# chanchanchan97/ICAFusion

Measured on AMD Instinct MI355X. Metric: RGB/IR image-pairs/sec (two-stream forward + NMS), higher is better.
Workload: dtype bf16

## Files before the change

### icafusion_amd/csrc/detect.hip

```cpp
#pragma clang fp contract(off)
#include "icaf_common.h"
#include "stream_core.h"
#include <cstdlib>

namespace icaf {

struct Anchors { float v[16]; };
int conv_prepare(const icaf_conv_args* a, ConvP& p);

struct DetectDiv { FastDiv no, nx, ny, na; };

template <bool I32>
__global__ __launch_bounds__(256) void detect_decode_kernel(const float* __restrict__ p, int ldp, float* __restrict__ z,
                                                            float* __restrict__ logits, float* __restrict__ raw, int B, int ny, int nx,
                                                            int na, int no, long long rows_total, long long row_offset, float stride,
                                                            Anchors anc, DetectDiv dv) {
    const long long total = (long long)B * na * ny * nx * no;
    for (long long e = (long long)blockIdx.x * blockDim.x + threadIdx.x; e < total; e += (long long)gridDim.x * blockDim.x) {
        int o, x, y, a, b;
        if constexpr (I32) {
            unsigned int q, r;
            fd_divmod((unsigned int)e, dv.no, q, r);
            o = (int)r;
            fd_divmod(q, dv.nx, q, r);
            x = (int)r;
            fd_divmod(q, dv.ny, q, r);
            y = (int)r;
            fd_divmod(q, dv.na, q, r);
            a = (int)r;
            b = (int)q;
        } else {
            o = (int)(e % no);
            const long long idx = e / no;
            x = (int)(idx % nx);
            long long t = idx / nx;
            y = (int)(t % ny);
            t /= ny;
            a = (int)(t % na);
            b = (int)(t / na);
        }
        const float v = p[(((long long)b * ny + y) * nx + x) * ldp + a * no + o];
        const long long row = (long long)b * rows_total + row_offset + ((long long)a * ny + y) * nx + x;
        if (raw) raw[e] = v;
        if (logits && o >= 5) logits[row * (no - 5) + (o - 5)] = v;
        const float sg = 1.0f / (1.0f + expf(-v));
        float out = sg;
        if (o == 0) out = ((sg * 2.0f - 0.5f) + (float)x) * stride;
        else if (o == 1) out = ((sg * 2.0f - 0.5f) + (float)y) * stride;
        else if (o == 2 || o == 3) {
            float an = anc.v[o - 2];
#pragma unroll
            for (int i = 1; i < 8; ++i) an = (a == i) ? (o == 2 ? anc.v[2 * i] : anc.v[2 * i + 1]) : an;
            const float d = sg * 2.0f;
            out = (d * d) * an;
        }
        z[row * no + o] = out;
    }
}

template <int NA, int NO>
__global__ __launch_bounds__(256) void detect_pixel_kernel(const float* __restrict__ p, int ldp, float* __restrict__ z,
                                                           float* __restrict__ logits, float* __restrict__ raw, int B, int ny, int nx,
                                                           long long rows_total, long long row_offset, float stride, Anchors anc,
                                                           FastDiv dnx, FastDiv dny) {
    constexpr int NV = NA * NO;
    const unsigned int total = (unsigned int)B * ny * nx;
    for (unsigned int pix = blockIdx.x * blockDim.x + threadIdx.x; pix < total; pix += gridDim.x * blockDim.x) {
        unsigned int t, x, b, y;
        fd_divmod(pix, dnx, t, x);
        fd_divmod(t, dny, b, y);
        const float* src = p + (long long)pix * ldp;
        float v[NV];
#pragma unroll
        for (int i = 0; i < NV; i += 2) {
            const float2 q = *(const float2*)(src + i);
            v[i] = q.x; v[i + 1] = q.y;
        }
#pragma unroll
        for (int a = 0; a < NA; ++a) {
            const long long cell = ((long long)a * ny + y) * nx + x;
            const long long row = (long long)b * rows_total + row_offset + cell;
            float o[NO];
#pragma unroll
            for (int k = 0; k < NO; ++k) {
                const float sg = 1.0f / (1.0f + expf(-v[a * NO + k]));
                float out = sg;
                if (k == 0) out = ((sg * 2.0f - 0.5f) + (float)x) * stride;
                else if (k == 1) out = ((sg * 2.0f - 0.5f) + (float)y) * stride;
                else if (k == 2 || k == 3) {
                    const float d = sg * 2.0f;
                    out = (d * d) * anc.v[2 * a + (k - 2)];
                }
                o[k] = out;
            }
            float* zr = z + row * NO;
#pragma unroll
            for (int k = 0; k < NO; k += 2) *(float2*)(zr + k) = float2{o[k], o[k + 1]};
            if (raw) {
                float* rr = raw + (((long long)b * NA) * ny * nx + cell) * NO;
#pragma unroll
                for (int k = 0; k < NO; k += 2) *(float2*)(rr + k) = float2{v[a * NO + k], v[a * NO + k + 1]};
            }
            if (logits) {
#pragma unroll
                for (int k = 5; k < NO; ++k) logits[row * (NO - 5) + (k - 5)] = v[a * NO + k];
            }
        }
    }
}

template <int NA, int NO>
static int launch_detect_pixel(const float* p, int ldp, float* z, float* logits, float* raw, int B, int ny, int nx, long long rows_total,
                               long long row_offset, float stride, const Anchors& anc, hipStream_t s) {
    const long long pixels = (long long)B * ny * nx;
    long long blocks = (pixels + 255) / 256;
    if (blocks > 256 * 32) blocks = 256 * 32;
    hipLaunchKernelGGL((detect_pixel_kernel<NA, NO>), dim3((unsigned)blocks), dim3(256), 0, s, p, ldp, z, logits, raw, B, ny, nx, rows_total,
                       row_offset, stride, anc, make_fastdiv((unsigned)nx), make_fastdiv((unsigned)ny));
    ICAF_LAUNCH_CHECK();
    return ICAF_OK;
}

template <int NA, int NO>
struct DetectEpi {
    static constexpr int SO = 64 * 4 + 16;
    float* z; float* logits; float* raw;
    int M, ny, nx; long long rows_total, row_offset; float stride; Anchors anc; FastDiv dnx, dny;
    template <int TM>
    __device__ __forceinline__ void stage(const f32x16 (&acc)[TM], const f32x4 (&bq)[4], unsigned char* stg, int row0, int col0, int l31, int hi, int, int) const {
#pragma unroll
        for (int qd = 0; qd < 4; ++qd) {
            const int nl = col0 + 8 * qd + 4 * hi;
#pragma unroll
            for (int b = 0; b < TM; ++b) {
                const int ml = row0 + b * 32 + l31;
                f32x4 v;
#pragma unroll
                for (int j = 0; j < 4; ++j) v[j] = acc[b][4 * qd + j] + bq[qd][j];
                *(f32x4*)(stg + ml * SO + nl * 4) = v;
            }
        }
    }
    __device__ __forceinline__ void flush(const unsigned char* stg, int m0, int n0, int tid) const {
        if (tid >= 128 * NA) return;
        const int row = tid / NA, a = tid - row * NA;
        const unsigned int pix = (unsigned int)(m0 + row);
        if ((int)pix >= M) return;
        unsigned int t, x, b, y;
        fd_divmod(pix, dnx, t, x);
        fd_divmod(t, dny, b, y);
        const float* src = (const float*)(stg + row * SO) + a * NO;
        float v[NO];
#pragma unroll
        for (int k = 0; k < NO; k += 2) { const float2 q2 = *(const float2*)(src + k); v[k] = q2.x; v[k + 1] = q2.y; }
        const long long cell = ((long long)a * ny + y) * nx + x;
        const long long zrow = (long long)b * rows_total + row_offset + cell;
        float o[NO];
#pragma unroll
        for (int k = 0; k < NO; ++k) {
            const float sg = 1.0f / (1.0f + expf(-v[k]));
            float out = sg;
            if (k == 0) out = ((sg * 2.0f - 0.5f) + (float)x) * stride;
            else if (k == 1) out = ((sg * 2.0f - 0.5f) + (float)y) * stride;
            else if (k == 2 || k == 3) {
                const float d = sg * 2.0f;
                out = (d * d) * anc.v[2 * a + (k - 2)];
            }
            o[k] = out;
        }
        float* zr = z + zrow * NO;
#pragma unroll
        for (int k = 0; k < NO; k += 2) *(float2*)(zr + k) = float2{o[k], o[k + 1]};
        if (raw) {
            float* rr = raw + (((long long)b * NA) * ny * nx + cell) * NO;
#pragma unroll
            for (int k = 0; k < NO; k += 2) *(float2*)(rr + k) = float2{v[k], v[k + 1]};
        }
        if (logits) {
#pragma unroll
            for (int k = 5; k < NO; ++k) logits[zrow * (NO - 5) + (k - 5)] = v[k];
        }
    }
};

template <int DT, int NA, int NO>
__global__ __launch_bounds__(512) void detect_conv_kernel(const ConvP p, const DetectEpi<NA, NO> epi) {
    stream_gemm<DT, 64, 1>(p, epi);
}

template <int DT, int NA, int NO>
static int launch_detect_conv(const ConvP& p, const DetectEpi<NA, NO>& epi, hipStream_t s) {
    constexpr int LDS = 3 * (128 + 64) * 128 + 128 * DetectEpi<NA, NO>::SO;
    ConvP q = p;
    q.mtiles = (p.M + 127) / 128;
    q.ntiles = 1;
    q.nchunks = p.K / 64;
    int dev = 0, cus = 256;
    ICAF_HIP(hipGetDevice(&dev));
    ICAF_HIP(hipDeviceGetAttribute(&cus, hipDeviceAttributeMultiprocessorCount, dev));
    const int grid = cus & ~7;
    ICAF_LDS_OPTIN((detect_conv_kernel<DT, NA, NO>), LDS);
    detect_conv_kernel<DT, NA, NO><<<dim3((unsigned)grid, 1, 1), dim3(512), LDS, s>>>(q, epi);
    ICAF_LAUNCH_CHECK();
    return ICAF_OK;
}

}

using namespace icaf;

enum { DETECT_PIXEL = 0, DETECT_ELEMENT = 1 };

static int detect_select(const float* p, int ldp, const float* z, const float* raw, int B, int ny, int nx, int na, int no) {
    const bool aligned = ldp % 2 == 0 && ((uintptr_t)p & 7) == 0 && ((uintptr_t)z & 7) == 0 && (!raw || ((uintptr_t)raw & 7) == 0);
    const bool pixel = na == 3 && (no == 6 || no == 8 || no == 14) && aligned && (long long)B * ny * nx < (1ll << 31) && !g_opt.detect_elementwise;
    return pixel ? DETECT_PIXEL : DETECT_ELEMENT;
}

extern "C" int icaf_detect_decode_kernel(const float* p, int ldp, const float* z, const float* raw, int B, int ny, int nx, int na, int no,
                                         int* kernel) {
    if (!p || !z || !kernel) return fail(ICAF_ERR_ARG, "icaf_detect_decode_kernel: null pointer");
    if (na < 1 || na > 8 || no < 6 || ldp < na * no) return fail(ICAF_ERR_ARG, "icaf_detect_decode_kernel: bad na/no/ldp");
    if (B < 1 || ny < 1 || nx < 1) return fail(ICAF_ERR_ARG, "icaf_detect_decode_kernel: empty level");
    *kernel = detect_select(p, ldp, z, raw, B, ny, nx, na, no);
    return ICAF_OK;
}

extern "C" int icaf_detect_decode(const float* p, int ldp, float* z, float* logits, float* raw, int B, int ny, int nx, int na, int no,
                                  long long rows_total, long long row_offset, float stride, const float* anchors_px, icaf_stream_t s) {
    if (!p || !z || !anchors_px) return fail(ICAF_ERR_ARG, "icaf_detect_decode: null pointer");
    if (na < 1 || na > 8 || no < 6 || ldp < na * no) return fail(ICAF_ERR_ARG, "icaf_detect_decode: bad na/no/ldp");
    if (row_offset + (long long)na * ny * nx > rows_total) return fail(ICAF_ERR_ARG, "icaf_detect_decode: level does not fit in z");
    Anchors anc;
    for (int i = 0; i < 16; ++i) anc.v[i] = i < 2 * na ? anchors_px[i] : 0.0f;
    const long long cells = (long long)B * na * ny * nx * no;
    long long blocks = (cells + 255) / 256;
    if (blocks > 256 * 32) blocks = 256 * 32;
    if (B < 1 || ny < 1 || nx < 1) return fail(ICAF_ERR_ARG, "icaf_detect_decode: empty level");
    if (detect_select(p, ldp, z, raw, B, ny, nx, na, no) == DETECT_PIXEL) {
        if (no == 6) return launch_detect_pixel<3, 6>(p, ldp, z, logits, raw, B, ny, nx, rows_total, row_offset, stride, anc, S(s));
        if (no == 8) return launch_detect_pixel<3, 8>(p, ldp, z, logits, raw, B, ny, nx, rows_total, row_offset, stride, anc, S(s));
        if (no == 14) return launch_detect_pixel<3, 14>(p, ldp, z, logits, raw, B, ny, nx, rows_total, row_offset, stride, anc, S(s));
    }
    const DetectDiv dv{make_fastdiv((unsigned)no), make_fastdiv((unsigned)nx), make_fastdiv((unsigned)ny), make_fastdiv((unsigned)na)};
    if (cells < (1ll << 31))
        hipLaunchKernelGGL(detect_decode_kernel<true>, dim3((unsigned)blocks), dim3(256), 0, S(s), p, ldp, z, logits, raw, B, ny, nx, na,
                           no, rows_total, row_offset, stride, anc, dv);
    else
        hipLaunchKernelGGL(detect_decode_kernel<false>, dim3((unsigned)blocks), dim3(256), 0, S(s), p, ldp, z, logits, raw, B, ny, nx, na,
                           no, rows_total, row_offset, stride, anc, dv);
    ICAF_LAUNCH_CHECK();
    return ICAF_OK;
}

extern "C" int icaf_detect_conv(const icaf_conv_args* a, float* z, float* logits, float* raw, int na, int no, long long rows_total,
                                long long row_offset, float stride, const float* anchors_px, icaf_stream_t s) {
    if (!a || !z || !anchors_px) return fail(ICAF_ERR_ARG, "icaf_detect_conv: null pointer");
    ConvP p;
    int st = conv_prepare(a, p);
    if (st) return st;
    if (a->dtype == ICAF_F32) return fail(ICAF_ERR_UNSUPPORTED, "icaf_detect_conv: 16-bit feature maps (the fp32 build runs icaf_conv2d + icaf_detect_decode)");
    if (a->kh != 1 || a->kw != 1 || a->sh != 1 || a->sw != 1 || a->ph || a->pw || a->groups != 1 || a->res || a->pre || a->w2 || a->act != ICAF_ACT_NONE)
        return fail(ICAF_ERR_ARG, "icaf_detect_conv: a plain 1x1 convolution without activation is expected");
    if ((a->Cin * 2) % 128 || p.x_bytes == 0) return fail(ICAF_ERR_UNSUPPORTED, "icaf_detect_conv: Cin * 2 bytes must be a multiple of 128 (Cin = %d)", a->Cin);
    if (na != 3 || (no != 6 && no != 8 && no != 14) || a->Cout != na * no) return fail(ICAF_ERR_UNSUPPORTED, "icaf_detect_conv: built for 3 anchors, no in {6, 8, 14} (na = %d, no = %d, Cout = %d)", na, no, a->Cout);
    if (row_offset + (long long)na * a->Ho * a->Wo > rows_total) return fail(ICAF_ERR_ARG, "icaf_detect_conv: level does not fit in z");
    if (((uintptr_t)z & 7) || (raw && ((uintptr_t)raw & 7))) return fail(ICAF_ERR_ARG, "icaf_detect_conv: z / raw must be 8-byte aligned");
    if ((long long)a->B * a->Ho * a->Wo >= (1ll << 31)) return fail(ICAF_ERR_UNSUPPORTED, "icaf_detect_conv: too many pixels");
    Anchors anc;
    for (int i = 0; i < 16; ++i) anc.v[i] = i < 2 * na ? anchors_px[i] : 0.0f;
    const FastDiv dnx = make_fastdiv((unsigned)a->Wo), dny = make_fastdiv((unsigned)a->Ho);
#define ICAF_DETECT_CONV(NO_)                                                                                                              \
    {                                                                                                                                      \
        DetectEpi<3, NO_> epi{z, logits, raw, p.M, a->Ho, a->Wo, rows_total, row_offset, stride, anc, dnx, dny};                           \
        return a->dtype == ICAF_BF16 ? launch_detect_conv<ICAF_BF16, 3, NO_>(p, epi, S(s)) : launch_detect_conv<ICAF_F16, 3, NO_>(p, epi, S(s)); \
    }
    if (no == 6) ICAF_DETECT_CONV(6)
    if (no == 8) ICAF_DETECT_CONV(8)
    ICAF_DETECT_CONV(14)
#undef ICAF_DETECT_CONV
}
```

### icafusion_amd/csrc/stream_core.h

```cpp
#pragma once
#include "conv_common.h"

namespace icaf {

template <int DT, int BN, int MODE, class EPI>
__device__ __forceinline__ void stream_gemm(const ConvP& p, const EPI& epi) {
    using E = Elem<DT>;
    static_assert(DT != ICAF_F32, "16-bit types");
    constexpr int BM = 128, RB = 128, NS = 3, NW = 8;
    constexpr int WN = 32, WM = BN == 128 ? 64 : 32;
    constexpr int TM = WM / 32, TN = 1;
    constexpr int WAVES_M = BM / WM;
    constexpr int VEC = E::VEC;
    constexpr int RPI = 8;
    constexpr int NA = BM / RPI / NW, NB = BN / RPI / NW;
    constexpr int PER = NA + NB;
    constexpr int STAGE = (BM + BN) * RB;
    constexpr int NSTEP = RB / 32;
    constexpr int RING = NS * STAGE;
    static_assert(NA >= 1 && NB >= 1 && (BN == 128 || BN == 64), "tile shape");
    extern __shared__ __attribute__((aligned(1024))) unsigned char lds[];
    unsigned char* stg = lds + RING;

    const int tid = threadIdx.x, lane = tid & 63, l31 = lane & 31, hi = lane >> 5;
    const int wave = __builtin_amdgcn_readfirstlane(tid >> 6);
    const int g = blockIdx.z;
    const int wm = wave % WAVES_M, wn = wave / WAVES_M;

    const __amdgpu_buffer_rsrc_t xr = __builtin_amdgcn_make_buffer_rsrc(
        (void*)((const typename E::type*)p.x + g * p.x_gs), 0, p.x_bytes, 0x00020000);
    const __amdgpu_buffer_rsrc_t wr = __builtin_amdgcn_make_buffer_rsrc(
        (void*)((const typename E::type*)p.w + g * p.w_gs), 0, p.w_bytes, 0x00020000);
    constexpr unsigned OOB = 0x80000000u;

    const int rsub = lane >> 3;
    const int dkey = ((wave & 1) << 2) | (rsub >> 1);
    const int lslot = (lane & 7) ^ dkey;

    const int xcd = blockIdx.x & 7, lb = blockIdx.x >> 3, wgx = gridDim.x >> 3;
    const int per_xcd = (p.mtiles + 7) >> 3, m_lo = xcd * per_xcd, m_hi = min(m_lo + per_xcd, p.mtiles);
    const int nt = lb % p.ntiles, mstride = wgx / p.ntiles, m_first = m_lo + lb / p.ntiles;
    const int n0 = nt * BN;
    const int nch = p.nchunks;

    int it = m_first, ic = 0;
    int kc = 0, ky = 0, kx = 0;
    unsigned ia_off[NA], iw_off[NB];
    int ia_h0[NA], ia_w0[NA];
#pragma unroll
    for (int i = 0; i < NB; ++i)
        iw_off[i] = ((unsigned)(n0 + (wave + NW * i) * RPI + rsub) * (unsigned)p.Kp + (unsigned)(lslot * VEC)) * E::BYTES;
    auto issue_setup = [&]() {
        const bool live = it < m_hi;
#pragma unroll
        for (int i = 0; i < NA; ++i) {
            const int m = it * BM + (wave + NW * i) * RPI + rsub;
            const bool ok = live && m < p.M;
            if constexpr (MODE == 1) {
                ia_off[i] = ok ? ((unsigned)m * (unsigned)p.ldx + (unsigned)(lslot * VEC)) * E::BYTES : OOB;
            } else {
                const int mm = ok ? m : 0;
                const int wo = mm % p.Wo, t = mm / p.Wo, ho = t % p.Ho, b = t / p.Ho;
                ia_h0[i] = ok ? ho * p.sh - p.ph : -0x10000;
                ia_w0[i] = wo * p.sw - p.pw;
                ia_off[i] = (unsigned)b * (unsigned)(p.H * p.W) * (unsigned)p.ldx * (unsigned)E::BYTES
                          + (unsigned)((ia_h0[i] * p.W + ia_w0[i]) * p.ldx + lslot * VEC) * E::BYTES;
            }
        }
    };
    auto issue_part = [&](int stage, int part) {
        unsigned char* st = lds + stage * STAGE;
        const unsigned koff = (unsigned)ic * RB;
        unsigned tap_delta = 0;
        if constexpr (MODE == 2) tap_delta = (unsigned)((ky * p.W + kx) * p.ldx + kc) * E::BYTES;
#pragma unroll
        for (int i = 0; i < NA; ++i) {
            if (i % NSTEP != part) continue;
            unsigned voff;
            if constexpr (MODE == 1) {
                voff = ia_off[i] == OOB ? OOB : ia_off[i] + koff;
            } else {
                const int h = ia_h0[i] + ky, w = ia_w0[i] + kx;
                const bool ok = (unsigned)h < (unsigned)p.H && (unsigned)w < (unsigned)p.W;
                voff = ok ? ia_off[i] + tap_delta : OOB;
            }
            __builtin_amdgcn_raw_ptr_buffer_load_lds(xr, (lds_ptr_t)(st + (wave + NW * i) * 1024), 16, voff, 0, 0, 0);
        }
#pragma unroll
        for (int i = 0; i < NB; ++i) {
            if ((NA + i) % NSTEP != part) continue;
            const unsigned voff = it < m_hi ? iw_off[i] + koff : OOB;
            __builtin_amdgcn_raw_ptr_buffer_load_lds(wr, (lds_ptr_t)(st + BM * RB + (wave + NW * i) * 1024), 16, voff, 0, 0, 0);
        }
    };
    auto issue_advance = [&]() {
        if constexpr (MODE == 2) {
            kc += RB / E::BYTES;
            if (kc >= p.Cin) { kc = 0; if (++kx == p.kw) { kx = 0; ++ky; } }
        }
        if (++ic == nch) {
            ic = 0; kc = 0; ky = 0; kx = 0;
            it += mstride;
            issue_setup();
        }
    };

    const float* __restrict__ bias = p.bias ? p.bias + g * p.bias_gs : nullptr;
    f32x4 bq[4];
#pragma unroll
    for (int qd = 0; qd < 4; ++qd) {
        const int n = n0 + wn * WN + 8 * qd + 4 * hi;
        const bool okn = bias && n < p.Cout;
        const float* bp = okn ? bias + n : (const float*)p.w;
        const f32x4 t = *(const f32x4*)bp;
        bq[qd] = okn ? t : f32x4{0.f, 0.f, 0.f, 0.f};
    }
#pragma unroll
    for (int qd = 0; qd < 4; ++qd) asm volatile("" : "+v"(bq[qd]));

    if (m_first >= m_hi) return;

    const int fkey = (l31 >> 1) & 7;
    int foff[NSTEP];
#pragma unroll
    for (int s = 0; s < NSTEP; ++s) foff[s] = l31 * RB + (((2 * s + hi) ^ fkey) << 4);

    issue_setup();
#pragma unroll
    for (int s = 0; s < NS; ++s) {
#pragma unroll
        for (int part = 0; part < NSTEP; ++part) issue_part(s, part);
        issue_advance();
    }

    int q = 0;
    for (int mt = m_first; mt < m_hi; mt += mstride) {
        const int m0 = mt * BM;
        f32x16 acc[TM];
#pragma unroll
        for (int b = 0; b < TM; ++b)
#pragma unroll
            for (int r = 0; r < 16; ++r) acc[b][r] = 0.0f;
        for (int c = 0; c < nch; ++c, ++q) {
            wait_vmcnt<PER>();
            asm volatile("s_waitcnt lgkmcnt(0)" ::: "memory");
            __builtin_amdgcn_s_barrier();
            const int sq = q % NS;
            const unsigned char* a_s = lds + sq * STAGE;
            const unsigned char* b_s = a_s + BM * RB;
            u32x4 fp[NSTEP][TM], fw[NSTEP];
#pragma unroll
            for (int s = 0; s < NSTEP; ++s) {
#pragma unroll
                for (int b = 0; b < TM; ++b) fp[s][b] = *(const u32x4*)(a_s + (wm * WM + b * 32) * RB + foff[s]);
                fw[s] = *(const u32x4*)(b_s + (wn * WN) * RB + foff[s]);
            }
            const int sfree = (q + NS - 1) % NS;
#pragma unroll
            for (int s = 0; s < NSTEP; ++s) {
#pragma unroll
                for (int b = 0; b < TM; ++b) mma_step<DT>(acc[b], fw[s], fp[s][b]);
                if (q > 0) issue_part(sfree, s);
            }
            if (q > 0) issue_advance();
        }

        epi.stage(acc, bq, stg, wm * WM, wn * WN, l31, hi, m0, n0);
        lds_barrier();
        epi.flush(stg, m0, n0, tid);
    }
    wait_vmcnt<0>();
}


}
```

Baseline: 16660.

## Narrow detect-head conv tile to BN=32 with 4 waves and two workgroups per CU

```diff
diff --git a/icafusion_amd/csrc/detect.hip b/icafusion_amd/csrc/detect.hip
--- a/icafusion_amd/csrc/detect.hip
+++ b/icafusion_amd/csrc/detect.hip
@@ -121,9 +121,34 @@
     return ICAF_OK;
 }
 
+typedef float detect_f2 __attribute__((ext_vector_type(2)));
+template <int NO>
+__device__ __forceinline__ void staged_read(const unsigned char* src, float (&v)[NO]) {
+    static_assert(NO == 6 || NO == 8 || NO == 14, "Detect heads built: no = 6 / 8 / 14");
+    const unsigned int ad = (unsigned int)(uintptr_t)(lds_ptr_t)src;
+    detect_f2 q[NO / 2];
+    if constexpr (NO == 6)
+        asm volatile("ds_read_b64 %0, %3\n\tds_read_b64 %1, %3 offset:8\n\tds_read_b64 %2, %3 offset:16\n\ts_waitcnt lgkmcnt(0)"
+                     : "=&v"(q[0]), "=&v"(q[1]), "=&v"(q[2]) : "v"(ad) : "memory");
+    else if constexpr (NO == 8)
+        asm volatile("ds_read_b64 %0, %4\n\tds_read_b64 %1, %4 offset:8\n\tds_read_b64 %2, %4 offset:16\n\tds_read_b64 %3, %4 offset:24\n\t"
+                     "s_waitcnt lgkmcnt(0)"
+                     : "=&v"(q[0]), "=&v"(q[1]), "=&v"(q[2]), "=&v"(q[3]) : "v"(ad) : "memory");
+    else
+        asm volatile("ds_read_b64 %0, %7\n\tds_read_b64 %1, %7 offset:8\n\tds_read_b64 %2, %7 offset:16\n\tds_read_b64 %3, %7 offset:24\n\t"
+                     "ds_read_b64 %4, %7 offset:32\n\tds_read_b64 %5, %7 offset:40\n\tds_read_b64 %6, %7 offset:48\n\ts_waitcnt lgkmcnt(0)"
+                     : "=&v"(q[0]), "=&v"(q[1]), "=&v"(q[2]), "=&v"(q[3]), "=&v"(q[4]), "=&v"(q[5]), "=&v"(q[6]) : "v"(ad) : "memory");
+#pragma unroll
+    for (int k = 0; k < NO / 2; ++k) { v[2 * k] = q[k][0]; v[2 * k + 1] = q[k][1]; }
+}
+
 template <int NA, int NO>
 struct DetectEpi {
-    static constexpr int SO = 64 * 4 + 16;
+    static constexpr int BN = NA * NO <= 32 ? 32 : 64;
+    static constexpr int NW = BN == 32 ? 4 : 8;
+    static constexpr int SO = BN * 4 + 16;
+    static constexpr int LDS = 3 * (128 + BN) * 128 + 128 * SO;
+    static constexpr int WGS_PER_CU = BN == 32 ? 2 : 1;
     float* z; float* logits; float* raw;
     int M, ny, nx; long long rows_total, row_offset; float stride; Anchors anc; FastDiv dnx, dny;
     template <int TM>
@@ -142,19 +167,25 @@
         }
     }
     __device__ __forceinline__ void flush(const unsigned char* stg, int m0, int n0, int tid) const {
-        if (tid >= 128 * NA) return;
-        const int row = tid / NA, a = tid - row * NA;
+#pragma unroll
+        for (int it0 = 0; it0 < 128 * NA; it0 += NW * 64) {
+            const int item = it0 + tid;
+            if (item < 128 * NA) flush_item(stg, m0, item & 127, item >> 7);
+        }
+    }
+    __device__ __forceinline__ void flush_item(const unsigned char* stg, int m0, int row, int a) const {
         const unsigned int pix = (unsigned int)(m0 + row);
         if ((int)pix >= M) return;
         unsigned int t, x, b, y;
         fd_divmod(pix, dnx, t, x);
         fd_divmod(t, dny, b, y);
-        const float* src = (const float*)(stg + row * SO) + a * NO;
         float v[NO];
-#pragma unroll
-        for (int k = 0; k < NO; k += 2) { const float2 q2 = *(const float2*)(src + k); v[k] = q2.x; v[k + 1] = q2.y; }
+        staged_read<NO>(stg + row * SO + a * NO * 4, v);
         const long long cell = ((long long)a * ny + y) * nx + x;
         const long long zrow = (long long)b * rows_total + row_offset + cell;
+        float aw = anc.v[0], ah = anc.v[1];
+#pragma unroll
+        for (int i = 1; i < NA; ++i) { aw = a == i ? anc.v[2 * i] : aw; ah = a == i ? anc.v[2 * i + 1] : ah; }
         float o[NO];
 #pragma unroll
         for (int k = 0; k < NO; ++k) {
@@ -164,7 +195,7 @@
             else if (k == 1) out = ((sg * 2.0f - 0.5f) + (float)y) * stride;
             else if (k == 2 || k == 3) {
                 const float d = sg * 2.0f;
-                out = (d * d) * anc.v[2 * a + (k - 2)];
+                out = (d * d) * (k == 2 ? aw : ah);
             }
             o[k] = out;
         }
@@ -184,13 +215,13 @@
 };
 
 template <int DT, int NA, int NO>
-__global__ __launch_bounds__(512) void detect_conv_kernel(const ConvP p, const DetectEpi<NA, NO> epi) {
-    stream_gemm<DT, 64, 1>(p, epi);
+__global__ __launch_bounds__((DetectEpi<NA, NO>::NW * 64)) void detect_conv_kernel(const ConvP p, const DetectEpi<NA, NO> epi) {
+    stream_gemm<DT, DetectEpi<NA, NO>::BN, 1, DetectEpi<NA, NO>::NW>(p, epi);
 }
 
 template <int DT, int NA, int NO>
 static int launch_detect_conv(const ConvP& p, const DetectEpi<NA, NO>& epi, hipStream_t s) {
-    constexpr int LDS = 3 * (128 + 64) * 128 + 128 * DetectEpi<NA, NO>::SO;
+    using EPI = DetectEpi<NA, NO>;
     ConvP q = p;
     q.mtiles = (p.M + 127) / 128;
     q.ntiles = 1;
@@ -198,9 +229,9 @@
     int dev = 0, cus = 256;
     ICAF_HIP(hipGetDevice(&dev));
     ICAF_HIP(hipDeviceGetAttribute(&cus, hipDeviceAttributeMultiprocessorCount, dev));
-    const int grid = cus & ~7;
-    ICAF_LDS_OPTIN((detect_conv_kernel<DT, NA, NO>), LDS);
-    detect_conv_kernel<DT, NA, NO><<<dim3((unsigned)grid, 1, 1), dim3(512), LDS, s>>>(q, epi);
+    const int grid = (cus * EPI::WGS_PER_CU) & ~7;
+    ICAF_LDS_OPTIN((detect_conv_kernel<DT, NA, NO>), EPI::LDS);
+    detect_conv_kernel<DT, NA, NO><<<dim3((unsigned)grid, 1, 1), dim3(EPI::NW * 64), EPI::LDS, s>>>(q, epi);
     ICAF_LAUNCH_CHECK();
     return ICAF_OK;
 }
diff --git a/icafusion_amd/csrc/stream_core.h b/icafusion_amd/csrc/stream_core.h
--- a/icafusion_amd/csrc/stream_core.h
+++ b/icafusion_amd/csrc/stream_core.h
@@ -3,11 +3,11 @@
 
 namespace icaf {
 
-template <int DT, int BN, int MODE, class EPI>
+template <int DT, int BN, int MODE, int NW = 8, class EPI>
 __device__ __forceinline__ void stream_gemm(const ConvP& p, const EPI& epi) {
     using E = Elem<DT>;
     static_assert(DT != ICAF_F32, "16-bit types");
-    constexpr int BM = 128, RB = 128, NS = 3, NW = 8;
+    constexpr int BM = 128, RB = 128, NS = 3;
     constexpr int WN = 32, WM = BN == 128 ? 64 : 32;
     constexpr int TM = WM / 32, TN = 1;
     constexpr int WAVES_M = BM / WM;
@@ -18,7 +18,8 @@
     constexpr int STAGE = (BM + BN) * RB;
     constexpr int NSTEP = RB / 32;
     constexpr int RING = NS * STAGE;
-    static_assert(NA >= 1 && NB >= 1 && (BN == 128 || BN == 64), "tile shape");
+    static_assert(NA >= 1 && NB >= 1 && NB * RPI * NW == BN && (BN == 128 || BN == 64 || BN == 32), "tile shape");
+    static_assert((BM / WM) * (BN / WN) == NW && NW % 2 == 0, "one 32-column accumulator block per wave; the DMA swizzle key needs an even wave count");
     extern __shared__ __attribute__((aligned(1024))) unsigned char lds[];
     unsigned char* stg = lds + RING;
 
```

After: 16740, median of 6. About the same (+0.5%).
